# michael-fonder/M4Depth

Hardware: AMD Instinct MI355X
Metric: frames/s (higher is better)
Workload: dtype f32

## Files before the change

### m4depth_amd/csrc/m4d_reduce.hip

```cpp
#include <cstdlib>
#include "m4d_common.h"
#include "../../include/m4depth_hip.h"

namespace {

constexpr int kDinlMaxBlocks = 512;
__host__ __device__ constexpr long long dinl_partial_floats(int b, int C) { return 2LL * b * kDinlMaxBlocks * C; }

__global__ void __launch_bounds__(256)
dinl_partial_kernel(const float* __restrict__ x, const float* __restrict__ mean, int hw, int C, int pass,
                    double* __restrict__ partial) {
  __shared__ double sh[4][256];
  const int bi = blockIdx.y;
  const int c4n = C >> 2;
  const int ppi = 256 / c4n;
  const int c4 = threadIdx.x % c4n, po = threadIdx.x / c4n;
  const float* xb = x + (long long)bi * hw * C;
  float4 m = make_float4(0.f, 0.f, 0.f, 0.f);
  if (pass == 1) m = *reinterpret_cast<const float4*>(mean + bi * C + c4 * 4);
  double acc[4] = {0.0, 0.0, 0.0, 0.0};
  for (int p = blockIdx.x * ppi + po; p < hw; p += gridDim.x * ppi) {
    float4 v = *reinterpret_cast<const float4*>(xb + (long long)p * C + c4 * 4);
    if (pass == 1) {
      v.x = v.x - m.x; v.y = v.y - m.y; v.z = v.z - m.z; v.w = v.w - m.w;
      v.x = v.x * v.x; v.y = v.y * v.y; v.z = v.z * v.z; v.w = v.w * v.w;
    }
    acc[0] += (double)v.x; acc[1] += (double)v.y; acc[2] += (double)v.z; acc[3] += (double)v.w;
  }
#pragma unroll
  for (int e = 0; e < 4; ++e) sh[e][threadIdx.x] = acc[e];
  __syncthreads();
  if (po == 0) {
    double* pp = partial + ((long long)bi * gridDim.x + blockIdx.x) * C + c4 * 4;
#pragma unroll
    for (int e = 0; e < 4; ++e) {
      double s = sh[e][c4];
      for (int r = 1; r < ppi; ++r) s += sh[e][r * c4n + c4];
      pp[e] = s;
    }
  }
}

__global__ void __launch_bounds__(256)
dinl_finalize_kernel(const double* __restrict__ partial, int nblk, int C, int hw, float* __restrict__ out) {
  __shared__ double sh[256];
  const int bi = blockIdx.x;
  const int c = threadIdx.x % C, j = threadIdx.x / C, nj = 256 / C;
  double s = 0.0;
  for (int k = j; k < nblk; k += nj) s += partial[((long long)bi * nblk + k) * C + c];
  sh[threadIdx.x] = s;
  __syncthreads();
  if (j == 0) {
    for (int r = 1; r < nj; ++r) s += sh[r * C + c];
    out[bi * C + c] = (float)(s / (double)hw);
  }
}

template <int C>
__global__ void __launch_bounds__(256)
dinl_apply_kernel(const float* __restrict__ x, const float* __restrict__ mean, const float* __restrict__ var,
                  const float* __restrict__ scale, const float* __restrict__ bias, int hw, int w, float slope,
                  float* __restrict__ out, int out_h, int out_w, int off_y, int off_x) {
  const int bi = blockIdx.y;
  float mu[C], dv[C], sc[C], bs[C];
#pragma unroll
  for (int c = 0; c < C; ++c) {
    mu[c] = mean[bi * C + c];
    dv[c] = var[bi * C + c] + 1e-12f;
    sc[c] = scale[c];
    bs[c] = bias[c];
  }
  for (int p = blockIdx.x * blockDim.x + threadIdx.x; p < hw; p += gridDim.x * blockDim.x) {
    const float* px = x + ((long long)bi * hw + p) * C;
    float n[C];
    float ss = 0.f;
#pragma unroll
    for (int c = 0; c < C; c += 4) {
      const float4 v = *reinterpret_cast<const float4*>(px + c);
      n[c] = (v.x - mu[c]) / dv[c]; n[c + 1] = (v.y - mu[c + 1]) / dv[c + 1];
      n[c + 2] = (v.z - mu[c + 2]) / dv[c + 2]; n[c + 3] = (v.w - mu[c + 3]) / dv[c + 3];
    }
#pragma unroll
    for (int c = 0; c < C; ++c) ss = ss + n[c] * n[c];
    const float inv = 1.0f / sqrtf(fmaxf(ss, 1e-12f));
    float* po = out + (((long long)bi * out_h + (p / w + off_y)) * out_w + (p % w + off_x)) * C;
#pragma unroll
    for (int c = 0; c < C; c += 4) {
      float4 o;
      o.x = sc[c] * (n[c] * inv) + bs[c]; o.y = sc[c + 1] * (n[c + 1] * inv) + bs[c + 1];
      o.z = sc[c + 2] * (n[c + 2] * inv) + bs[c + 2]; o.w = sc[c + 3] * (n[c + 3] * inv) + bs[c + 3];
      o.x = o.x > 0.f ? o.x : o.x * slope; o.y = o.y > 0.f ? o.y : o.y * slope;
      o.z = o.z > 0.f ? o.z : o.z * slope; o.w = o.w > 0.f ? o.w : o.w * slope;
      *reinterpret_cast<float4*>(po + c) = o;
    }
  }
}

template <int C>
__global__ void __launch_bounds__(256)
enc_head_conv_kernel(const float* __restrict__ img, const float* __restrict__ w27, const float* __restrict__ bias,
                     int h, int w, int bsz, long long stride_b, long long stride_t,
                     float* __restrict__ out, double* __restrict__ partial) {
  __shared__ double sh[4][C];
  const int bi = blockIdx.y;
  const int hw = h * w;
  const float* ib = img + (long long)(bi % bsz) * stride_b + (long long)(bi / bsz) * stride_t;
  float* ob = out + (long long)bi * hw * C;
  double csum[C];
#pragma unroll
  for (int c = 0; c < C; ++c) csum[c] = 0.0;
  for (int p = blockIdx.x * 256 + threadIdx.x; p < hw; p += gridDim.x * 256) {
    const int y = p / w, x = p - y * w;
    typedef float f2 __attribute__((ext_vector_type(2)));
    f2 acc2[C / 2];
#pragma unroll
    for (int c = 0; c < C / 2; ++c) acc2[c] = (f2){0.f, 0.f};
#pragma unroll
    for (int ky = 0; ky < 3; ++ky) {
      const int yy = y + ky - 1;
#pragma unroll
      for (int kx = 0; kx < 3; ++kx) {
        const int xx = x + kx - 1;
        const bool in = yy >= 0 && yy < h && xx >= 0 && xx < w;
        const float* px = ib + ((long long)(in ? yy : y) * w + (in ? xx : x)) * 3;
        const float v0 = in ? px[0] : 0.f, v1 = in ? px[1] : 0.f, v2 = in ? px[2] : 0.f;
        const f2* wt = reinterpret_cast<const f2*>(w27 + (ky * 3 + kx) * 3 * C);
#pragma unroll
        for (int c = 0; c < C / 2; ++c)
          acc2[c] = ((acc2[c] + (f2){v0, v0} * wt[c]) + (f2){v1, v1} * wt[C / 2 + c]) + (f2){v2, v2} * wt[C + c];
      }
    }
    float acc[C];
#pragma unroll
    for (int c = 0; c < C / 2; ++c) { acc[2 * c] = acc2[c].x; acc[2 * c + 1] = acc2[c].y; }
#pragma unroll
    for (int c = 0; c < C; c += 4) {
      float4 o = make_float4(acc[c] + bias[c], acc[c + 1] + bias[c + 1], acc[c + 2] + bias[c + 2], acc[c + 3] + bias[c + 3]);
      *reinterpret_cast<float4*>(ob + (long long)p * C + c) = o;
      csum[c] += (double)o.x; csum[c + 1] += (double)o.y; csum[c + 2] += (double)o.z; csum[c + 3] += (double)o.w;
    }
  }
#pragma unroll
  for (int c = 0; c < C; ++c) {
    double v = csum[c];
#pragma unroll
    for (int o = 32; o > 0; o >>= 1) v += __shfl_xor(v, o);
    if ((threadIdx.x & 63) == 0) sh[threadIdx.x >> 6][c] = v;
  }
  __syncthreads();
  if (threadIdx.x < C)
    partial[((long long)bi * gridDim.x + blockIdx.x) * C + threadIdx.x] =
        ((sh[0][threadIdx.x] + sh[1][threadIdx.x]) + sh[2][threadIdx.x]) + sh[3][threadIdx.x];
}

constexpr int kMetricSums = 9;
constexpr int kMetricBlocks = 512;

__global__ void __launch_bounds__(256)
metrics_partial_kernel(const float* __restrict__ gt_raw, const float* __restrict__ est_raw, long long n, float max_d,
                       double* __restrict__ partial, long long per_image, long long gt_image_stride) {
  float s[kMetricSums];
#pragma unroll
  for (int k = 0; k < kMetricSums; ++k) s[k] = 0.f;
  const long long step = (long long)gridDim.x * blockDim.x;
  long long i = (long long)blockIdx.x * blockDim.x + threadIdx.x;
  long long img = i / per_image, off = i - img * per_image;
  for (; i < n; i += step) {
    const float gt = fminf(fmaxf(gt_raw[img * gt_image_stride + off], 0.0f), max_d);
    off += step;
    while (off >= per_image) { off -= per_image; ++img; }
    const float est = fminf(fmaxf(est_raw[i], 0.001f), max_d);
    const bool m = gt > 1e-6f;
    const float diff = gt - est;
    const float lg = logf(gt + 1e-6f), le = logf(est + 1e-6f);
    const bool m2 = lg > 1e-6f;
    const float th = fmaxf(gt / est, est / gt);
    if (m) {
      s[0] += 1.0f;
      s[1] += fabsf(diff) / (gt + 1e-6f);
      s[2] += diff * diff / (gt + 1e-6f);
      s[3] += diff * diff;
      s[6] += th < 1.25f ? 1.0f : 0.0f;
      s[7] += th < 1.5625f ? 1.0f : 0.0f;
      s[8] += th < 1.953125f ? 1.0f : 0.0f;
    }
    if (m2) { s[4] += 1.0f; s[5] += (lg - le) * (lg - le); }
  }
  __shared__ double sh[4][kMetricSums];
#pragma unroll
  for (int k = 0; k < kMetricSums; ++k) {
    double v = (double)s[k];
#pragma unroll
    for (int o = 32; o > 0; o >>= 1) v += __shfl_down(v, o);
    if ((threadIdx.x & 63) == 0) sh[threadIdx.x >> 6][k] = v;
  }
  __syncthreads();
  if (threadIdx.x < kMetricSums)
    partial[(long long)blockIdx.x * kMetricSums + threadIdx.x] =
        ((sh[0][threadIdx.x] + sh[1][threadIdx.x]) + sh[2][threadIdx.x]) + sh[3][threadIdx.x];
}

__global__ void __launch_bounds__(kMetricSums * 32)
metrics_finalize_kernel(const double* __restrict__ partial, int nblk, float* __restrict__ out7,
                        float* __restrict__ total7, float count, float* __restrict__ mean7) {
  __shared__ double sub[kMetricSums * 32];
  __shared__ double tot[kMetricSums];
  const int q = threadIdx.x % kMetricSums, j = threadIdx.x / kMetricSums;
  double s = 0.0;
  for (int k = j; k < nblk; k += 32) s += partial[(long long)k * kMetricSums + q];
  sub[threadIdx.x] = s;
  __syncthreads();
  if (j == 0) {
    for (int r = 1; r < 32; ++r) s += sub[r * kMetricSums + q];
    tot[q] = s;
  }
  __syncthreads();
  if (threadIdx.x == 0) {
    const double cnt = tot[0] > 1.0 ? tot[0] : 1.0, cnt2 = tot[4] > 1.0 ? tot[4] : 1.0;
    out7[0] = (float)(tot[1] / cnt);
    out7[1] = (float)(tot[2] / cnt);
    out7[2] = sqrtf((float)(tot[3] / cnt));
    out7[3] = sqrtf((float)(tot[5] / cnt2));
    out7[4] = (float)(tot[6] / cnt);
    out7[5] = (float)(tot[7] / cnt);
    out7[6] = (float)(tot[8] / cnt);
    if (total7) {
#pragma unroll
      for (int i = 0; i < 7; ++i) {
        const float t = total7[i] + out7[i];
        total7[i] = t;
        if (mean7) mean7[i] = t / count;
      }
    }
  }
}

__global__ void __launch_bounds__(256)
metrics_partial_ps_kernel(const float* __restrict__ gt_raw, long long gt_stride, const float* __restrict__ est_raw,
                          long long est_stride, long long n, float max_d, double* __restrict__ partial) {
  const float* gt_img = gt_raw + (long long)blockIdx.y * gt_stride;
  const float* est_img = est_raw + (long long)blockIdx.y * est_stride;
  float s[kMetricSums];
#pragma unroll
  for (int k = 0; k < kMetricSums; ++k) s[k] = 0.f;
  const long long step = (long long)gridDim.x * blockDim.x;
  for (long long i = (long long)blockIdx.x * blockDim.x + threadIdx.x; i < n; i += step) {
    const float gt = fminf(fmaxf(gt_img[i], 0.0f), max_d);
    const float est = fminf(fmaxf(est_img[i], 0.001f), max_d);
    const bool m = gt > 1e-6f;
    const float diff = gt - est;
    const float lg = logf(gt + 1e-6f), le = logf(est + 1e-6f);
    const bool m2 = lg > 1e-6f;
    const float th = fmaxf(gt / est, est / gt);
    if (m) {
      s[0] += 1.0f;
      s[1] += fabsf(diff) / (gt + 1e-6f);
      s[2] += diff * diff / (gt + 1e-6f);
      s[3] += diff * diff;
      s[6] += th < 1.25f ? 1.0f : 0.0f;
      s[7] += th < 1.5625f ? 1.0f : 0.0f;
      s[8] += th < 1.953125f ? 1.0f : 0.0f;
    }
    if (m2) { s[4] += 1.0f; s[5] += (lg - le) * (lg - le); }
  }
  __shared__ double sh[4][kMetricSums];
#pragma unroll
  for (int k = 0; k < kMetricSums; ++k) {
    double v = (double)s[k];
#pragma unroll
    for (int o = 32; o > 0; o >>= 1) v += __shfl_down(v, o);
    if ((threadIdx.x & 63) == 0) sh[threadIdx.x >> 6][k] = v;
  }
  __syncthreads();
  if (threadIdx.x < kMetricSums)
    partial[((long long)blockIdx.y * gridDim.x + blockIdx.x) * kMetricSums + threadIdx.x] =
        ((sh[0][threadIdx.x] + sh[1][threadIdx.x]) + sh[2][threadIdx.x]) + sh[3][threadIdx.x];
}

__global__ void __launch_bounds__(kMetricSums * 32)
metrics_finalize_ps_kernel(const double* __restrict__ partial, int nblk, const unsigned char* __restrict__ new_traj,
                           const unsigned char* __restrict__ active, float* __restrict__ rows, unsigned char* __restrict__ counted) {
  __shared__ double sub[kMetricSums * 32];
  __shared__ double tot[kMetricSums];
  const int smp = blockIdx.x;
  const double* pp = partial + (long long)smp * nblk * kMetricSums;
  const int q = threadIdx.x % kMetricSums, j = threadIdx.x / kMetricSums;
  double s = 0.0;
  for (int k = j; k < nblk; k += 32) s += pp[(long long)k * kMetricSums + q];
  sub[threadIdx.x] = s;
  __syncthreads();
  if (j == 0) {
    for (int r = 1; r < 32; ++r) s += sub[r * kMetricSums + q];
    tot[q] = s;
  }
  __syncthreads();
  if (threadIdx.x == 0) {
    const double cnt = tot[0] > 1.0 ? tot[0] : 1.0, cnt2 = tot[4] > 1.0 ? tot[4] : 1.0;
    float* out7 = rows + (long long)smp * 7;
    out7[0] = (float)(tot[1] / cnt);
    out7[1] = (float)(tot[2] / cnt);
    out7[2] = sqrtf((float)(tot[3] / cnt));
    out7[3] = sqrtf((float)(tot[5] / cnt2));
    out7[4] = (float)(tot[6] / cnt);
    out7[5] = (float)(tot[7] / cnt);
    out7[6] = (float)(tot[8] / cnt);
    counted[smp] = (active[smp] != 0 && new_traj[smp] == 0) ? 1 : 0;
  }
}


typedef float f32x4 __attribute__((ext_vector_type(4)));

__device__ __forceinline__ void enc0_lane_setup(const float* __restrict__ w27, int lane, int row_stride, int (&koff)[7], float (&wb)[7]) {
  const int j = lane & 15, g = lane >> 4;
#pragma unroll
  for (int s = 0; s < 7; ++s) {
    const int k = 4 * s + g;
    const bool valid = k < 27;
    const int kk = valid ? k : 0;
    koff[s] = (kk / 9) * row_stride + kk % 9;
    wb[s] = valid ? w27[k * 16 + j] : 0.f;
  }
}
__device__ __forceinline__ f32x4 enc0_conv1(const float* window_base, const int (&koff)[7], const float (&wb)[7]) {
  f32x4 acc = {0.f, 0.f, 0.f, 0.f};
#pragma unroll
  for (int s = 0; s < 7; ++s) acc = __builtin_amdgcn_mfma_f32_16x16x4f32(window_base[koff[s]], wb[s], acc, 0, 0, 0);
  return acc;
}

constexpr int kE0TW = 128, kE0TH = 8;
constexpr int kE0RS = (kE0TW + 2) * 3;

__device__ __forceinline__ float enc0_shift(const float* __restrict__ ib, const float* __restrict__ w27, const float* __restrict__ bias,
                                            int h, int w, int j) {
  const int cy = h / 2, cx = w / 2;
  float y = bias[j];
  for (int ky = 0; ky < 3; ++ky)
    for (int kx = 0; kx < 3; ++kx) {
      const int gy = cy + ky - 1, gx = cx + kx - 1;
      if (gy < 0 || gy >= h || gx < 0 || gx >= w) continue;
      for (int ch = 0; ch < 3; ++ch) y = y + w27[((ky * 3 + kx) * 3 + ch) * 16 + j] * ib[((long long)gy * w + gx) * 3 + ch];
    }
  return y;
}

template <int PASS>
__global__ void __launch_bounds__(256)
enc0_stats_kernel(const float* __restrict__ img, const float* __restrict__ w27, const float* __restrict__ bias,
                  const float* __restrict__ mean, int h, int w, int bsz, long long stride_b, long long stride_t,
                  int tiles_x, int n_tiles, double* __restrict__ partial) {
  __shared__ float tile[(kE0TH + 2) * kE0RS];
  __shared__ double sh[2][4][16];
  const int t = threadIdx.x, lane = t & 63, wv = t >> 6;
  const int j = lane & 15, g = lane >> 4;
  const int bi = blockIdx.y;
  const float* ib = img + (long long)(bi % bsz) * stride_b + (long long)(bi / bsz) * stride_t;
  int koff[7]; float wb[7];
  enc0_lane_setup(w27, lane, kE0RS, koff, wb);
  const float bias_j = bias[j];
  const float mean_j = PASS == 1 ? mean[bi * 16 + j] : (PASS == 2 ? enc0_shift(ib, w27, bias, h, w, j) : 0.f);
  const double shift_j = (double)mean_j;
  double csum = 0.0, csum2 = 0.0;
  for (int ti = blockIdx.x; ti < n_tiles; ti += gridDim.x) {
    const int y0 = (ti / tiles_x) * kE0TH, x0 = (ti % tiles_x) * kE0TW;
    __syncthreads();
    for (int idx = t; idx < (kE0TH + 2) * kE0RS; idx += 256) {
      const int r = idx / kE0RS, cc = idx - r * kE0RS;
      const int gy = y0 - 1 + r, gxc = (x0 - 1) * 3 + cc;
      const bool in = gy >= 0 && gy < h && gxc >= 0 && gxc < w * 3;
      tile[idx] = in ? ib[(long long)gy * w * 3 + gxc] : 0.f;
    }
    __syncthreads();
#pragma unroll
    for (int rr = 0; rr < 2; ++rr) {
      const int yl = 2 * wv + rr;
#pragma unroll
      for (int ct = 0; ct < kE0TW / 16; ++ct) {
        const f32x4 acc = enc0_conv1(tile + yl * kE0RS + 3 * (16 * ct + j), koff, wb);
#pragma unroll
        for (int r = 0; r < 4; ++r) {
          const bool valid = y0 + yl < h && x0 + 16 * ct + 4 * g + r < w;
          float v = acc[r] + bias_j;
          if (PASS == 1) { v = v - mean_j; v = v * v; }
          if (PASS == 2) {
            const double d = valid ? (double)v - shift_j : 0.0;
            csum += d;
            csum2 = fma(d, d, csum2);
          } else {
            csum += valid ? (double)v : 0.0;
          }
        }
      }
    }
  }
  csum += __shfl_xor(csum, 16);
  csum += __shfl_xor(csum, 32);
  if (PASS == 2) {
    csum2 += __shfl_xor(csum2, 16);
    csum2 += __shfl_xor(csum2, 32);
  }
  if (lane < 16) { sh[0][wv][lane] = csum; sh[1][wv][lane] = csum2; }
  __syncthreads();
  constexpr int NQ = PASS == 2 ? 32 : 16;
  if (t < NQ) {
    const int q = t >> 4, c = t & 15;
    partial[((long long)bi * gridDim.x + blockIdx.x) * NQ + t] = ((sh[q][0][c] + sh[q][1][c]) + sh[q][2][c]) + sh[q][3][c];
  }
}

__global__ void __launch_bounds__(256)
enc0_moments_finalize_kernel(const float* __restrict__ img, const double* __restrict__ partial, int nblk, const float* __restrict__ w27,
                             const float* __restrict__ bias, int h, int w, int bsz, long long stride_b, long long stride_t,
                             float* __restrict__ mean, float* __restrict__ var) {
  __shared__ double sh[256];
  const int bi = blockIdx.x, t = threadIdx.x;
  const int c = t & 31, j = t >> 5;
  double pv[32];
  const int cnt = (nblk - j + 7) / 8;
#pragma unroll
  for (int i = 0; i < 32; ++i) pv[i] = i < cnt ? partial[((long long)bi * nblk + j + 8 * i) * 32 + c] : 0.0;
  __shared__ float s_shift[16];
  if (t >= 240) {
    const float* ib0 = img + (long long)(bi % bsz) * stride_b + (long long)(bi / bsz) * stride_t;
    s_shift[t - 240] = enc0_shift(ib0, w27, bias, h, w, t - 240);
  }
  double s = 0.0;
#pragma unroll
  for (int i = 0; i < 32; ++i) s += pv[i];
  sh[t] = s;
  __syncthreads();
  if (t < 32) {
    for (int r = 1; r < 8; ++r) s += sh[r * 32 + t];
    sh[t] = s;
  }
  __syncthreads();
  if (t < 16) {
    const double n = (double)h * (double)w;
    const double m1 = sh[t] / n, m2 = sh[16 + t] / n;
    mean[bi * 16 + t] = (float)((double)s_shift[t] + m1);
    const double v = m2 - m1 * m1;
    var[bi * 16 + t] = (float)(v > 0.0 ? v : 0.0);
  }
}

__global__ void __launch_bounds__(256)
enc0_rgb_total_kernel(const float* __restrict__ img, int hw, int bsz, long long stride_b, long long stride_t, float* __restrict__ partial) {
  __shared__ float sh[4][3];
  const int t = threadIdx.x, bi = blockIdx.y;
  const float* ib = img + (long long)(bi % bsz) * stride_b + (long long)(bi / bsz) * stride_t;
  float s0 = 0.f, s1 = 0.f, s2 = 0.f;
  for (int p = blockIdx.x * 256 + t; p < hw; p += gridDim.x * 256) {
    s0 += ib[(long long)p * 3]; s1 += ib[(long long)p * 3 + 1]; s2 += ib[(long long)p * 3 + 2];
  }
#pragma unroll
  for (int o = 32; o > 0; o >>= 1) { s0 += __shfl_xor(s0, o); s1 += __shfl_xor(s1, o); s2 += __shfl_xor(s2, o); }
  if ((t & 63) == 0) { sh[t >> 6][0] = s0; sh[t >> 6][1] = s1; sh[t >> 6][2] = s2; }
  __syncthreads();
  if (t < 3) partial[((long long)bi * gridDim.x + blockIdx.x) * 3 + t] = ((sh[0][t] + sh[1][t]) + sh[2][t]) + sh[3][t];
}

__global__ void __launch_bounds__(256)
enc0_mean_kernel(const float* __restrict__ img, const float* __restrict__ partial, int nblk, const float* __restrict__ w27,
                 const float* __restrict__ bias, int h, int w, int bsz, long long stride_b, long long stride_t, float* __restrict__ mean) {
  __shared__ double red[15][256];
  __shared__ double sums[3][5];
  const int t = threadIdx.x, bi = blockIdx.x;
  const float* ib = img + (long long)(bi % bsz) * stride_b + (long long)(bi / bsz) * stride_t;
  double acc[15];
#pragma unroll
  for (int q = 0; q < 15; ++q) acc[q] = 0.0;
  for (int k = t; k < nblk; k += 256)
#pragma unroll
    for (int ch = 0; ch < 3; ++ch) acc[ch * 5] += (double)partial[((long long)bi * nblk + k) * 3 + ch];
  for (int x = t; x < w; x += 256)
#pragma unroll
    for (int ch = 0; ch < 3; ++ch) {
      acc[ch * 5 + 1] += (double)ib[(long long)x * 3 + ch];
      acc[ch * 5 + 2] += (double)ib[((long long)(h - 1) * w + x) * 3 + ch];
    }
  for (int y = t; y < h; y += 256)
#pragma unroll
    for (int ch = 0; ch < 3; ++ch) {
      acc[ch * 5 + 3] += (double)ib[((long long)y * w) * 3 + ch];
      acc[ch * 5 + 4] += (double)ib[((long long)y * w + (w - 1)) * 3 + ch];
    }
#pragma unroll
  for (int q = 0; q < 15; ++q) red[q][t] = acc[q];
  __syncthreads();
  for (int o = 128; o > 0; o >>= 1) {
    if (t < o)
#pragma unroll
      for (int q = 0; q < 15; ++q) red[q][t] += red[q][t + o];
    __syncthreads();
  }
  if (t < 15) sums[t / 5][t % 5] = red[t][0];
  __syncthreads();
  if (t < 16) {
    double m = 0.0;
    for (int ky = 0; ky < 3; ++ky)
      for (int kx = 0; kx < 3; ++kx)
        for (int ch = 0; ch < 3; ++ch) {
          const int ry = ky == 0 ? h - 1 : (ky == 2 ? 0 : -1), cx = kx == 0 ? w - 1 : (kx == 2 ? 0 : -1);
          double sv = sums[ch][0];
          if (ry >= 0) sv -= sums[ch][ry == 0 ? 1 : 2];
          if (cx >= 0) sv -= sums[ch][cx == 0 ? 3 : 4];
          if (ry >= 0 && cx >= 0) sv += (double)ib[((long long)ry * w + cx) * 3 + ch];
          m += (double)w27[((ky * 3 + kx) * 3 + ch) * 16 + t] * sv;
        }
    mean[bi * 16 + t] = (float)((double)bias[t] + m / ((double)h * (double)w));
  }
}

#ifndef M4D_E0_ABL
#define M4D_E0_ABL 0
#endif
constexpr int kF0OW = 16, kF0OH = 8;
constexpr int kF0CW = 2 * kF0OW + 1, kF0CH = 2 * kF0OH + 1;
constexpr int kF0RW = kF0CW + 2, kF0RH = kF0CH + 2;
constexpr int kF0RS = kF0RW * 3;
constexpr int kF0NS = 17;
constexpr int kF0NP = kF0CW * kF0CH;

__device__ __forceinline__ bool v_dummy(float x) { return x != 1.2345e-30f; }
__global__ void __launch_bounds__(256)
enc0_fused_kernel(const float* __restrict__ img, const float* __restrict__ w27, const float* __restrict__ bias1,
                  const float* __restrict__ mean, const float* __restrict__ var, const float* __restrict__ dn_scale,
                  const float* __restrict__ dn_bias, float dn_slope, const float* __restrict__ w2, const float* __restrict__ bias2,
                  float slope, int h, int w, int oh, int ow, int pad_y, int pad_x, int bsz, long long stride_b, long long stride_t,
                  int tiles_x, float* __restrict__ out) {
  __shared__ float rgb[kF0RH * kF0RS];
  __shared__ float nrm[kF0NP * kF0NS];
  const int t = threadIdx.x, lane = t & 63, wv = t >> 6;
  const int j = lane & 15, g = lane >> 4;
  const int bi = blockIdx.y;
  const float* ib = img + (long long)(bi % bsz) * stride_b + (long long)(bi / bsz) * stride_t;
  const int oy0 = (blockIdx.x / tiles_x) * kF0OH, ox0 = (blockIdx.x % tiles_x) * kF0OW;
  const int cy0 = 2 * oy0 - pad_y, cx0 = 2 * ox0 - pad_x;
  for (int idx = t; idx < kF0RH * kF0RS; idx += 256) {
    const int r = idx / kF0RS, cc = idx - r * kF0RS;
    const int gy = cy0 - 1 + r, gxc = (cx0 - 1) * 3 + cc;
    const bool in = gy >= 0 && gy < h && gxc >= 0 && gxc < w * 3;
    rgb[idx] = (in && !(M4D_E0_ABL & 1)) ? ib[(long long)gy * w * 3 + gxc] : 0.f;
  }
  int koff[7]; float wb[7];
  enc0_lane_setup(w27, lane, kF0RS, koff, wb);
  const float bias_j = bias1[j];
  __shared__ float s_mu[16], s_dv[16], s_sc[16], s_bs[16];
  if (t < 16) {
    s_mu[t] = mean[bi * 16 + t];
    s_dv[t] = 1.0f / (var[bi * 16 + t] + 1e-12f);
    s_sc[t] = dn_scale[t]; s_bs[t] = dn_bias[t];
  }
  float wb2[36];
#pragma unroll
  for (int s = 0; s < 36; ++s) wb2[s] = w2[(4 * s + g) * 16 + j];
  const float bias2_j = bias2[j];
  __syncthreads();
  static_assert((kF0NP + 15) / 16 == 36, "nine 16-pixel tiles per wave");
#pragma unroll 3
  for (int it = 0; it < 9; ++it) {
    const int tl = wv + 4 * it;
    const int pa = min(16 * tl + j, kF0NP - 1);
    const int ay = pa / kF0CW, ax = pa - ay * kF0CW;
    const f32x4 acc = (M4D_E0_ABL & 2) ? f32x4{wb[0], wb[1], wb[2], wb[3]} : enc0_conv1(rgb + ay * kF0RS + 3 * ax, koff, wb);
#pragma unroll
    for (int r = 0; r < 4; ++r) {
      const int p = 16 * tl + 4 * g + r;
      if (p < kF0NP) nrm[p * kF0NS + j] = acc[r] + bias_j;
    }
  }
  __syncthreads();
  for (int p = t; p < ((M4D_E0_ABL & 4) ? 0 : kF0NP); p += 256) {
    const int py = p / kF0CW, px = p - py * kF0CW;
    const bool inside = cy0 + py >= 0 && cy0 + py < h && cx0 + px >= 0 && cx0 + px < w;
    float* q = nrm + p * kF0NS;
    float n[16];
    float ss = 0.f;
#pragma unroll
    for (int c = 0; c < 16; ++c) { n[c] = (q[c] - s_mu[c]) * s_dv[c]; ss = ss + n[c] * n[c]; }
    const float inv = 1.0f / sqrtf(fmaxf(ss, 1e-12f));
#pragma unroll
    for (int c = 0; c < 16; ++c) {
      float o = s_sc[c] * (n[c] * inv) + s_bs[c];
      o = o > 0.f ? o : o * dn_slope;
      q[c] = inside ? o : 0.f;
    }
  }
  __syncthreads();
#pragma unroll
  for (int rr = 0; rr < 2; ++rr) {
    const int oyl = 2 * wv + rr;
    const float* base = nrm + ((2 * oyl) * kF0CW + 2 * j) * kF0NS + g;
    f32x4 acc = {0.f, 0.f, 0.f, 0.f};
#pragma unroll
    for (int s = 0; s < ((M4D_E0_ABL & 8) ? 1 : 36); ++s) {
      const int tap = s >> 2, ky = tap / 3, kx = tap - 3 * ky;
      acc = __builtin_amdgcn_mfma_f32_16x16x4f32(base[(ky * kF0CW + kx) * kF0NS + 4 * (s & 3)], wb2[s], acc, 0, 0, 0);
    }
    const int oy = oy0 + oyl;
#pragma unroll
    for (int r = 0; r < 4; ++r) {
      const int ox = ox0 + 4 * g + r;
      if (oy < oh && ox < ow && !((M4D_E0_ABL & 16) && v_dummy(acc[r]))) {
        float v = acc[r] + bias2_j;
        v = v > 0.f ? v : v * slope;
        out[(((long long)bi * oh + oy) * ow + ox) * 16 + j] = v;
      }
    }
  }
}

}

extern "C" long long m4d_dinl_workspace_floats(int b, int C) {
  return dinl_partial_floats(b, C) + 2LL * b * C;
}

extern "C" int m4d_dinl_fwd(const float* x, const float* scale, const float* bias, int b, int h, int w, int C,
                            float slope, float* workspace, float* out, void* stream) {
  return m4d_dinl_fwd_padded(x, scale, bias, b, h, w, C, slope, workspace, out, h, w, 0, 0, stream);
}

extern "C" int m4d_dinl_fwd_padded(const float* x, const float* scale, const float* bias, int b, int h, int w, int C,
                                   float slope, float* workspace, float* out, int out_h, int out_w, int off_y,
                                   int off_x, void* stream) {
  M4D_CHECK_ARG(x && scale && bias && workspace && out && b > 0 && h > 0 && w > 0);
  M4D_CHECK_ARG(off_y >= 0 && off_x >= 0 && off_y + h <= out_h && off_x + w <= out_w);
  M4D_CHECK_ARG(C == 16 || C == 32);
  M4D_CHECK_ARG(((((uintptr_t)x | (uintptr_t)out | (uintptr_t)workspace)) & 15u) == 0);
  hipStream_t s = (hipStream_t)stream;
  const int hw = h * w;
  const int ppi = 256 / (C / 4);
  int nblk = (hw + ppi * 8 - 1) / (ppi * 8);
  if (nblk > kDinlMaxBlocks) nblk = kDinlMaxBlocks;
  double* partial = reinterpret_cast<double*>(workspace);
  float* mean = workspace + dinl_partial_floats(b, C);
  float* var = mean + (long long)b * C;
  m4d_launch(dinl_partial_kernel, dim3(nblk, b), dim3(256), 0, s, x, (const float*)nullptr, hw, C, 0, partial);
  m4d_launch(dinl_finalize_kernel, dim3(b), dim3(256), 0, s, (const double*)partial, nblk, C, hw, mean);
  m4d_launch(dinl_partial_kernel, dim3(nblk, b), dim3(256), 0, s, x, (const float*)mean, hw, C, 1, partial);
  m4d_launch(dinl_finalize_kernel, dim3(b), dim3(256), 0, s, (const double*)partial, nblk, C, hw, var);
  int gx = m4d_blocks(hw, 256);
  if (gx > 2048) gx = 2048;
  if (C == 16) m4d_launch(dinl_apply_kernel<16>, dim3(gx, b), dim3(256), 0, s, x, mean, var, scale, bias, hw, w, slope, out, out_h, out_w, off_y, off_x);
  else m4d_launch(dinl_apply_kernel<32>, dim3(gx, b), dim3(256), 0, s, x, mean, var, scale, bias, hw, w, slope, out, out_h, out_w, off_y, off_x);
  return M4D_LAUNCH_RESULT();
}

extern "C" int m4d_enc_head_fwd(const float* images, int bsz, long long stride_b, long long stride_t,
                                const float* w_hwio, const float* bias, int b, int h, int w, int C,
                                float* workspace, float* raw_out, void* stream) {
  M4D_CHECK_ARG(images && w_hwio && bias && workspace && raw_out && b > 0 && h > 0 && w > 0);
  M4D_CHECK_ARG(C == 16);
  M4D_CHECK_ARG(bsz > 0 && b % bsz == 0 && stride_b >= 0 && stride_t >= 0);
  M4D_CHECK_ARG(((((uintptr_t)raw_out | (uintptr_t)workspace)) & 15u) == 0);
  hipStream_t s = (hipStream_t)stream;
  const int hw = h * w;
  int nblk = (hw + 256 * 8 - 1) / (256 * 8);
  if (nblk > kDinlMaxBlocks) nblk = kDinlMaxBlocks;
  if (nblk < 1) nblk = 1;
  double* partial = reinterpret_cast<double*>(workspace);
  float* mean = workspace + dinl_partial_floats(b, C);
  float* var = mean + (long long)b * C;
  m4d_launch(enc_head_conv_kernel<16>, dim3(nblk, b), dim3(256), 0, s, images, w_hwio, bias, h, w, bsz, stride_b, stride_t,
                     raw_out, partial);
  m4d_launch(dinl_finalize_kernel, dim3(b), dim3(256), 0, s, (const double*)partial, nblk, C, hw, mean);
  const int ppi = 256 / (C / 4);
  int nblk2 = (hw + ppi * 8 - 1) / (ppi * 8);
  if (nblk2 > kDinlMaxBlocks) nblk2 = kDinlMaxBlocks;
  m4d_launch(dinl_partial_kernel, dim3(nblk2, b), dim3(256), 0, s, (const float*)raw_out, (const float*)mean, hw, C, 1, partial);
  m4d_launch(dinl_finalize_kernel, dim3(b), dim3(256), 0, s, (const double*)partial, nblk2, C, hw, var);
  return M4D_LAUNCH_RESULT();
}

extern "C" int m4d_enc_level0_stats(const float* images, int bsz, long long stride_b, long long stride_t,
                                    const float* w1_hwio, const float* bias1, int b, int h, int w, float* workspace,
                                    float* mean, float* var, void* stream) {
  M4D_CHECK_ARG(images && w1_hwio && bias1 && workspace && mean && var);
  M4D_CHECK_ARG(b > 0 && h > 0 && w > 0 && bsz > 0 && b % bsz == 0 && stride_b >= 0 && stride_t >= 0);
  M4D_CHECK_ARG((((uintptr_t)workspace) & 7u) == 0);
  hipStream_t s = (hipStream_t)stream;
  const int C = 16, hw = h * w;
  const int tiles_x = (w + kE0TW - 1) / kE0TW, n_tiles = tiles_x * ((h + kE0TH - 1) / kE0TH);
  const int nblk = n_tiles < kDinlMaxBlocks ? n_tiles : kDinlMaxBlocks;
  double* partial = reinterpret_cast<double*>(workspace);
  static const int single_pass = [] { const char* e = getenv("M4D_ENC0_SINGLE_PASS"); return e ? atoi(e) : 1; }();
  static const int analytic_mean_env = [] { const char* e = getenv("M4D_ENC0_ANALYTIC_MEAN"); return e ? atoi(e) : 1; }();
  if (single_pass) {
    const int cap = kDinlMaxBlocks / 2, per = (n_tiles + cap - 1) / cap;
    const int nb2 = (n_tiles + per - 1) / per;
    m4d_launch(enc0_stats_kernel<2>, dim3(nb2, b), dim3(256), 0, s, images, w1_hwio, bias1, (const float*)nullptr, h, w, bsz,
               stride_b, stride_t, tiles_x, n_tiles, partial);
    m4d_launch(enc0_moments_finalize_kernel, dim3(b), dim3(256), 0, s, images, (const double*)partial, nb2, w1_hwio, bias1, h, w, bsz,
               stride_b, stride_t, mean, var);
    return M4D_LAUNCH_RESULT();
  }
  const bool analytic_mean = analytic_mean_env && h > 1 && w > 1;
  if (analytic_mean) {
    int nb3 = (hw + 256 * 16 - 1) / (256 * 16);
    if (nb3 > kDinlMaxBlocks) nb3 = kDinlMaxBlocks;
    m4d_launch(enc0_rgb_total_kernel, dim3(nb3, b), dim3(256), 0, s, images, hw, bsz, stride_b, stride_t, workspace);
    m4d_launch(enc0_mean_kernel, dim3(b), dim3(256), 0, s, images, (const float*)workspace, nb3, w1_hwio, bias1, h, w, bsz,
                       stride_b, stride_t, mean);
  } else {
    m4d_launch(enc0_stats_kernel<0>, dim3(nblk, b), dim3(256), 0, s, images, w1_hwio, bias1, (const float*)nullptr, h, w, bsz,
                       stride_b, stride_t, tiles_x, n_tiles, partial);
    m4d_launch(dinl_finalize_kernel, dim3(b), dim3(256), 0, s, (const double*)partial, nblk, C, hw, mean);
  }
  m4d_launch(enc0_stats_kernel<1>, dim3(nblk, b), dim3(256), 0, s, images, w1_hwio, bias1, (const float*)mean, h, w, bsz,
                     stride_b, stride_t, tiles_x, n_tiles, partial);
  m4d_launch(dinl_finalize_kernel, dim3(b), dim3(256), 0, s, (const double*)partial, nblk, C, hw, var);
  return M4D_LAUNCH_RESULT();
}

extern "C" int m4d_enc_level0_apply(const float* images, int bsz, long long stride_b, long long stride_t,
                                    const float* w1_hwio, const float* bias1, const float* mean, const float* var,
                                    const float* dn_scale, const float* dn_bias, float dn_slope, const float* w2_hwio,
                                    const float* bias2, float slope, int b, int h, int w, float* out, void* stream) {
  M4D_CHECK_ARG(images && w1_hwio && bias1 && mean && var && dn_scale && dn_bias && w2_hwio && bias2 && out);
  M4D_CHECK_ARG(b > 0 && h > 0 && w > 0 && bsz > 0 && b % bsz == 0 && stride_b >= 0 && stride_t >= 0);
  const int oh = (h + 1) / 2, ow = (w + 1) / 2;
  const int ftx = (ow + kF0OW - 1) / kF0OW, fty = (oh + kF0OH - 1) / kF0OH;
  const int tot_y = (oh - 1) * 2 + 3 - h, tot_x = (ow - 1) * 2 + 3 - w;
  const int pad_y = (tot_y > 0 ? tot_y : 0) / 2, pad_x = (tot_x > 0 ? tot_x : 0) / 2;
  m4d_launch(enc0_fused_kernel, dim3(ftx * fty, b), dim3(256), 0, (hipStream_t)stream, images, w1_hwio, bias1, mean,
                     var, dn_scale, dn_bias, dn_slope, w2_hwio, bias2, slope, h, w, oh, ow, pad_y, pad_x, bsz, stride_b,
                     stride_t, ftx, out);
  return M4D_LAUNCH_RESULT();
}

extern "C" int m4d_enc_level0_fwd(const float* images, int bsz, long long stride_b, long long stride_t,
                                   const float* w1_hwio, const float* bias1, const float* dn_scale, const float* dn_bias,
                                   float dn_slope, const float* w2_hwio, const float* bias2, float slope,
                                   int b, int h, int w, float* workspace, float* out, void* stream) {
  M4D_CHECK_ARG(workspace && b > 0);
  float* mean = workspace + dinl_partial_floats(b, 16);
  float* var = mean + (long long)b * 16;
  const int rc = m4d_enc_level0_stats(images, bsz, stride_b, stride_t, w1_hwio, bias1, b, h, w, workspace, mean, var, stream);
  if (rc != 0) return rc;
  return m4d_enc_level0_apply(images, bsz, stride_b, stride_t, w1_hwio, bias1, mean, var, dn_scale, dn_bias, dn_slope, w2_hwio,
                              bias2, slope, b, h, w, out, stream);
}

extern "C" long long m4d_metrics_workspace_bytes(void) { return (long long)kMetricBlocks * kMetricSums * sizeof(double); }

extern "C" int m4d_depth_metrics_strided(const float* gt, long long per_image, long long gt_image_stride, const float* est,
                                         long long n, float max_d, void* workspace, float* out7, float* total7, float count,
                                         float* mean7, void* stream) {
  M4D_CHECK_ARG(gt && est && workspace && out7 && n > 0 && per_image > 0 && gt_image_stride >= per_image && n % per_image == 0);
  M4D_CHECK_ARG(!mean7 || (total7 && count > 0.f));
  hipStream_t s = (hipStream_t)stream;
  long long g = (n + 255) / 256;
  const int nblk = (int)(g < kMetricBlocks ? g : kMetricBlocks);
  m4d_launch(metrics_partial_kernel, dim3(nblk), dim3(256), 0, s, gt, est, n, max_d, (double*)workspace, per_image, gt_image_stride);
  m4d_launch(metrics_finalize_kernel, dim3(1), dim3(kMetricSums * 32), 0, s, (const double*)workspace, nblk, out7, total7, count, mean7);
  return M4D_LAUNCH_RESULT();
}

extern "C" int m4d_depth_metrics(const float* gt, const float* est, long long n, float max_d, void* workspace,
                                 float* out7, float* total7, float count, float* mean7, void* stream) {
  return m4d_depth_metrics_strided(gt, n, n, est, n, max_d, workspace, out7, total7, count, mean7, stream);
}

extern "C" long long m4d_metrics_per_sample_workspace_bytes(int b) {
  return b > 0 ? (long long)b * kMetricBlocks * kMetricSums * sizeof(double) : 0;
}

extern "C" int m4d_depth_metrics_per_sample(const float* gt, long long gt_stride, const float* est, long long est_stride,
                                            int b, long long per_image, float max_d, const unsigned char* new_traj,
                                            const unsigned char* active, void* workspace, float* rows, unsigned char* counted,
                                            void* stream) {
  M4D_CHECK_ARG(gt && est && new_traj && active && workspace && rows && counted);
  M4D_CHECK_ARG(b > 0 && b <= 65535 && per_image > 0 && gt_stride >= per_image && est_stride >= per_image);
  hipStream_t s = (hipStream_t)stream;
  long long g = (per_image + 255) / 256;
  const int nblk = (int)(g < kMetricBlocks ? g : kMetricBlocks);
  m4d_launch(metrics_partial_ps_kernel, dim3(nblk, b), dim3(256), 0, s, gt, gt_stride, est, est_stride, per_image, max_d,
             (double*)workspace);
  m4d_launch(metrics_finalize_ps_kernel, dim3(b), dim3(kMetricSums * 32), 0, s, (const double*)workspace, nblk, new_traj, active,
             rows, counted);
  return M4D_LAUNCH_RESULT();
}
```

Before: 1791.

## Double-buffer enc0 stats tiles and interleave MFMA chains in fused first layer

The stats kernel now double-buffers its shared-memory input tile. Each thread prefetches the next tile's pixels into registers while the current tile's MFMA convolution runs, which removes one barrier per iteration, and a compile-time fast path skips the bounds checks for interior tiles. The shift computation is split into a load phase and a sum phase so its global loads are issued early, and the finalize kernel computes the shift in every thread instead of a separate branch. In the fused encoder kernel, global loads go into registers before the stores to LDS, three independent MFMA chains are interleaved in the first conv, and the second conv's two rows are computed together with software-prefetched LDS operands and scheduling barriers. The cost is higher register pressure, which could reduce occupancy.

Result: faster. 1814 (median of 6 runs) (+1.3%).

```diff
diff --git a/m4depth_amd/csrc/m4d_reduce.hip b/m4depth_amd/csrc/m4d_reduce.hip
--- a/m4depth_amd/csrc/m4d_reduce.hip
+++ b/m4depth_amd/csrc/m4d_reduce.hip
@@ -1,3 +1,4 @@
+#include <type_traits>
 #include <cstdlib>
 #include "m4d_common.h"
 #include "../../include/m4depth_hip.h"
@@ -329,20 +330,66 @@
   return acc;
 }
 
+#ifndef M4D_E0S_ABL
+#define M4D_E0S_ABL 0
+#endif
 constexpr int kE0TW = 128, kE0TH = 8;
 constexpr int kE0RS = (kE0TW + 2) * 3;
 
-__device__ __forceinline__ float enc0_shift(const float* __restrict__ ib, const float* __restrict__ w27, const float* __restrict__ bias,
-                                            int h, int w, int j) {
+__device__ __forceinline__ void enc0_shift_load(const float* __restrict__ ib, const float* __restrict__ w27, int h, int w, int j,
+                                                float (&sw)[27], float (&sp)[27]) {
   const int cy = h / 2, cx = w / 2;
-  float y = bias[j];
+#pragma unroll
   for (int ky = 0; ky < 3; ++ky)
+#pragma unroll
     for (int kx = 0; kx < 3; ++kx) {
       const int gy = cy + ky - 1, gx = cx + kx - 1;
-      if (gy < 0 || gy >= h || gx < 0 || gx >= w) continue;
-      for (int ch = 0; ch < 3; ++ch) y = y + w27[((ky * 3 + kx) * 3 + ch) * 16 + j] * ib[((long long)gy * w + gx) * 3 + ch];
+      const bool ok = !(gy < 0 || gy >= h || gx < 0 || gx >= w);
+      const long long base = ok ? ((long long)gy * w + gx) * 3 : 0LL;
+#pragma unroll
+      for (int ch = 0; ch < 3; ++ch) {
+        sw[(ky * 3 + kx) * 3 + ch] = w27[((ky * 3 + kx) * 3 + ch) * 16 + j];
+        sp[(ky * 3 + kx) * 3 + ch] = ib[base + ch];
+      }
+    }
+}
+__device__ __forceinline__ float enc0_shift_sum(float bias_j, const float (&sw)[27], const float (&sp)[27], int h, int w) {
+  const int cy = h / 2, cx = w / 2;
+  float y = bias_j;
+#pragma unroll
+  for (int ky = 0; ky < 3; ++ky)
+#pragma unroll
+    for (int kx = 0; kx < 3; ++kx) {
+      const int gy = cy + ky - 1, gx = cx + kx - 1;
+      const bool ok = !(gy < 0 || gy >= h || gx < 0 || gx >= w);
+#pragma unroll
+      for (int ch = 0; ch < 3; ++ch) y = ok ? y + sw[(ky * 3 + kx) * 3 + ch] * sp[(ky * 3 + kx) * 3 + ch] : y;
     }
   return y;
+}
+
+constexpr int kE0TE = (kE0TH + 2) * kE0RS;
+constexpr int kE0NL = (kE0TE + 255) / 256;
+static_assert(kE0RS > 256 && kE0RS < 512, "enc0_tile_load: thread t starts in row 0 and crosses at most one row end per step of 256");
+__device__ __forceinline__ unsigned enc0_tile_load(const float* __restrict__ ib, int h, int w, int y0, int x0, int t, float (&v)[kE0NL]) {
+  const int row3 = w * 3, gy0 = y0 - 1, gc0 = (x0 - 1) * 3;
+  int r = 0, cc = t;
+  unsigned mask = 0u;
+#pragma unroll
+  for (int i = 0; i < kE0NL; ++i) {
+    const int gy = gy0 + r, gxc = gc0 + cc;
+    const bool in = r < kE0TH + 2 && gy >= 0 && gy < h && gxc >= 0 && gxc < row3;
+    v[i] = ib[(long long)min(max(gy, 0), h - 1) * row3 + min(max(gxc, 0), row3 - 1)];
+    mask |= in ? 1u << i : 0u;
+    cc += 256;
+    if (cc >= kE0RS) { cc -= kE0RS; ++r; }
+  }
+  return mask;
+}
+__device__ __forceinline__ void enc0_tile_store(float* __restrict__ tile, int t, const float (&v)[kE0NL], unsigned mask) {
+#pragma unroll
+  for (int i = 0; i < kE0NL; ++i)
+    if (t + 256 * i < kE0TE) tile[t + 256 * i] = (mask >> i & 1u) ? v[i] : 0.f;
 }
 
 template <int PASS>
@@ -350,49 +397,65 @@
 enc0_stats_kernel(const float* __restrict__ img, const float* __restrict__ w27, const float* __restrict__ bias,
                   const float* __restrict__ mean, int h, int w, int bsz, long long stride_b, long long stride_t,
                   int tiles_x, int n_tiles, double* __restrict__ partial) {
-  __shared__ float tile[(kE0TH + 2) * kE0RS];
+  __shared__ float tile[2][kE0TE];
   __shared__ double sh[2][4][16];
   const int t = threadIdx.x, lane = t & 63, wv = t >> 6;
   const int j = lane & 15, g = lane >> 4;
   const int bi = blockIdx.y;
   const float* ib = img + (long long)(bi % bsz) * stride_b + (long long)(bi / bsz) * stride_t;
+  float v[kE0NL];
+  int ti = blockIdx.x;
+  unsigned vmask = 0u;
+  if (ti < n_tiles) vmask = enc0_tile_load(ib, h, w, (ti / tiles_x) * kE0TH, (ti % tiles_x) * kE0TW, t, v);
+  float sw[27], sp[27];
+  if (PASS == 2) enc0_shift_load(ib, w27, h, w, j, sw, sp);
   int koff[7]; float wb[7];
   enc0_lane_setup(w27, lane, kE0RS, koff, wb);
   const float bias_j = bias[j];
-  const float mean_j = PASS == 1 ? mean[bi * 16 + j] : (PASS == 2 ? enc0_shift(ib, w27, bias, h, w, j) : 0.f);
+  const float mean_j = PASS == 1 ? mean[bi * 16 + j] : (PASS == 2 ? enc0_shift_sum(bias_j, sw, sp, h, w) : 0.f);
   const double shift_j = (double)mean_j;
   double csum = 0.0, csum2 = 0.0;
-  for (int ti = blockIdx.x; ti < n_tiles; ti += gridDim.x) {
+  if (ti < n_tiles) enc0_tile_store(tile[0], t, v, vmask);
+  __syncthreads();
+  int cur = 0;
+  for (; ti < n_tiles; ti += gridDim.x) {
     const int y0 = (ti / tiles_x) * kE0TH, x0 = (ti % tiles_x) * kE0TW;
-    __syncthreads();
-    for (int idx = t; idx < (kE0TH + 2) * kE0RS; idx += 256) {
-      const int r = idx / kE0RS, cc = idx - r * kE0RS;
-      const int gy = y0 - 1 + r, gxc = (x0 - 1) * 3 + cc;
-      const bool in = gy >= 0 && gy < h && gxc >= 0 && gxc < w * 3;
-      tile[idx] = in ? ib[(long long)gy * w * 3 + gxc] : 0.f;
-    }
-    __syncthreads();
-#pragma unroll
-    for (int rr = 0; rr < 2; ++rr) {
-      const int yl = 2 * wv + rr;
-#pragma unroll
-      for (int ct = 0; ct < kE0TW / 16; ++ct) {
-        const f32x4 acc = enc0_conv1(tile + yl * kE0RS + 3 * (16 * ct + j), koff, wb);
-#pragma unroll
-        for (int r = 0; r < 4; ++r) {
-          const bool valid = y0 + yl < h && x0 + 16 * ct + 4 * g + r < w;
-          float v = acc[r] + bias_j;
-          if (PASS == 1) { v = v - mean_j; v = v * v; }
-          if (PASS == 2) {
-            const double d = valid ? (double)v - shift_j : 0.0;
-            csum += d;
-            csum2 = fma(d, d, csum2);
-          } else {
-            csum += valid ? (double)v : 0.0;
+    const int tn = ti + gridDim.x;
+    const bool more = tn < n_tiles;
+    if (more) vmask = enc0_tile_load(ib, h, w, (tn / tiles_x) * kE0TH, (tn % tiles_x) * kE0TW, t, v);
+    const float* tb = tile[cur];
+    auto tile_sums = [&](auto whole) {
+      constexpr bool kWhole = decltype(whole)::value;
+#pragma unroll 1
+      for (int rr = 0; rr < 2; ++rr) {
+        const int yl = 2 * wv + rr;
+#pragma unroll 4
+        for (int ct = 0; ct < kE0TW / 16; ++ct) {
+          const float* wnd = tb + yl * kE0RS + 3 * (16 * ct + j);
+          const f32x4 acc = (M4D_E0S_ABL & 2) ? f32x4{wnd[koff[0]], wnd[koff[1]], wnd[koff[2]], wnd[koff[3]]} : enc0_conv1(wnd, koff, wb);
+#pragma unroll
+          for (int r = 0; r < 4; ++r) {
+            const bool valid = kWhole || (y0 + yl < h && x0 + 16 * ct + 4 * g + r < w);
+            float v1 = acc[r] + bias_j;
+            if (M4D_E0S_ABL & 4) { csum += r == 0 ? (double)v1 : 0.0; continue; }
+            if (PASS == 1) { v1 = v1 - mean_j; v1 = v1 * v1; }
+            if (PASS == 2) {
+              const double d = valid ? (double)v1 - shift_j : 0.0;
+              csum += d;
+              csum2 = fma(d, d, csum2);
+            } else {
+              csum += valid ? (double)v1 : 0.0;
+            }
           }
         }
       }
-    }
+    };
+    if (y0 + kE0TH <= h && x0 + kE0TW <= w) tile_sums(std::true_type{}); else tile_sums(std::false_type{});
+    if (more) {
+      enc0_tile_store(tile[cur ^ 1], t, v, vmask);
+      __syncthreads();
+    }
+    cur ^= 1;
   }
   csum += __shfl_xor(csum, 16);
   csum += __shfl_xor(csum, 32);
@@ -416,15 +479,18 @@
   __shared__ double sh[256];
   const int bi = blockIdx.x, t = threadIdx.x;
   const int c = t & 31, j = t >> 5;
+  const float* ib0 = img + (long long)(bi % bsz) * stride_b + (long long)(bi / bsz) * stride_t;
+  float sw[27], sp[27];
+  enc0_shift_load(ib0, w27, h, w, t & 15, sw, sp);
+  const float sbias = bias[t & 15];
   double pv[32];
   const int cnt = (nblk - j + 7) / 8;
 #pragma unroll
-  for (int i = 0; i < 32; ++i) pv[i] = i < cnt ? partial[((long long)bi * nblk + j + 8 * i) * 32 + c] : 0.0;
-  __shared__ float s_shift[16];
-  if (t >= 240) {
-    const float* ib0 = img + (long long)(bi % bsz) * stride_b + (long long)(bi / bsz) * stride_t;
-    s_shift[t - 240] = enc0_shift(ib0, w27, bias, h, w, t - 240);
-  }
+  for (int i = 0; i < 32; ++i) {
+    const double x = partial[i < cnt ? ((long long)bi * nblk + j + 8 * i) * 32 + c : 0LL];
+    pv[i] = i < cnt ? x : 0.0;
+  }
+  const float shift = enc0_shift_sum(sbias, sw, sp, h, w);
   double s = 0.0;
 #pragma unroll
   for (int i = 0; i < 32; ++i) s += pv[i];
@@ -438,7 +504,7 @@
   if (t < 16) {
     const double n = (double)h * (double)w;
     const double m1 = sh[t] / n, m2 = sh[16 + t] / n;
-    mean[bi * 16 + t] = (float)((double)s_shift[t] + m1);
+    mean[bi * 16 + t] = (float)((double)shift + m1);
     const double v = m2 - m1 * m1;
     var[bi * 16 + t] = (float)(v > 0.0 ? v : 0.0);
   }
@@ -537,37 +603,74 @@
   const float* ib = img + (long long)(bi % bsz) * stride_b + (long long)(bi / bsz) * stride_t;
   const int oy0 = (blockIdx.x / tiles_x) * kF0OH, ox0 = (blockIdx.x % tiles_x) * kF0OW;
   const int cy0 = 2 * oy0 - pad_y, cx0 = 2 * ox0 - pad_x;
-  for (int idx = t; idx < kF0RH * kF0RS; idx += 256) {
-    const int r = idx / kF0RS, cc = idx - r * kF0RS;
-    const int gy = cy0 - 1 + r, gxc = (cx0 - 1) * 3 + cc;
-    const bool in = gy >= 0 && gy < h && gxc >= 0 && gxc < w * 3;
-    rgb[idx] = (in && !(M4D_E0_ABL & 1)) ? ib[(long long)gy * w * 3 + gxc] : 0.f;
+  constexpr int kNL = (kF0RH * kF0RS + 255) / 256, kStep = 256 - 2 * kF0RS;
+  static_assert(kStep >= 0 && kStep < kF0RS && 3 * kF0RS > 256, "the row / column walk below");
+  float sv[kNL];
+  {
+    const int row3 = w * 3, gy0 = cy0 - 1, gc0 = (cx0 - 1) * 3;
+    int r = (t >= kF0RS) + (t >= 2 * kF0RS), cc = t - r * kF0RS;
+#pragma unroll
+    for (int i = 0; i < kNL; ++i) {
+      const int gy = gy0 + r, gxc = gc0 + cc;
+      const bool in = r < kF0RH && gy >= 0 && gy < h && gxc >= 0 && gxc < row3 && !(M4D_E0_ABL & 1);
+      const float x = ib[in ? (long long)gy * row3 + gxc : 0LL];
+      sv[i] = in ? x : 0.f;
+      r += 2; cc += kStep;
+      if (cc >= kF0RS) { cc -= kF0RS; ++r; }
+    }
   }
   int koff[7]; float wb[7];
   enc0_lane_setup(w27, lane, kF0RS, koff, wb);
   const float bias_j = bias1[j];
   __shared__ float s_mu[16], s_dv[16], s_sc[16], s_bs[16];
-  if (t < 16) {
-    s_mu[t] = mean[bi * 16 + t];
-    s_dv[t] = 1.0f / (var[bi * 16 + t] + 1e-12f);
-    s_sc[t] = dn_scale[t]; s_bs[t] = dn_bias[t];
-  }
+  const float st_mu = mean[bi * 16 + (t & 15)], st_var = var[bi * 16 + (t & 15)], st_sc = dn_scale[t & 15], st_bs = dn_bias[t & 15];
   float wb2[36];
 #pragma unroll
   for (int s = 0; s < 36; ++s) wb2[s] = w2[(4 * s + g) * 16 + j];
   const float bias2_j = bias2[j];
-  __syncthreads();
-  static_assert((kF0NP + 15) / 16 == 36, "nine 16-pixel tiles per wave");
-#pragma unroll 3
-  for (int it = 0; it < 9; ++it) {
-    const int tl = wv + 4 * it;
-    const int pa = min(16 * tl + j, kF0NP - 1);
-    const int ay = pa / kF0CW, ax = pa - ay * kF0CW;
-    const f32x4 acc = (M4D_E0_ABL & 2) ? f32x4{wb[0], wb[1], wb[2], wb[3]} : enc0_conv1(rgb + ay * kF0RS + 3 * ax, koff, wb);
+#pragma unroll
+  for (int i = 0; i < kNL; ++i)
+    if (t + 256 * i < kF0RH * kF0RS) rgb[t + 256 * i] = sv[i];
+  if (t < 16) {
+    s_mu[t] = st_mu;
+    s_dv[t] = 1.0f / (st_var + 1e-12f);
+    s_sc[t] = st_sc; s_bs[t] = st_bs;
+  }
+  __syncthreads();
+  static_assert((kF0NP + 15) / 16 == 36 && kF0NP > 16 * 35, "nine 16-pixel tiles per wave, the last one of wave 3 ragged");
+#pragma unroll 1
+  for (int it = 0; it < 9; it += 3) {
+    const float* wa[3];
+#pragma unroll
+    for (int u = 0; u < 3; ++u) {
+      const int pa = min(16 * (wv + 4 * (it + u)) + j, kF0NP - 1);
+      const int ay = pa / kF0CW, ax = pa - ay * kF0CW;
+      wa[u] = rgb + ay * kF0RS + 3 * ax;
+    }
+    f32x4 c0 = {0.f, 0.f, 0.f, 0.f}, c1 = c0, c2 = c0;
+    if (M4D_E0_ABL & 2) {
+      c0 = c1 = c2 = f32x4{wb[0], wb[1], wb[2], wb[3]};
+    } else {
+#pragma unroll
+      for (int s = 0; s < 7; ++s) {
+        c0 = __builtin_amdgcn_mfma_f32_16x16x4f32(wa[0][koff[s]], wb[s], c0, 0, 0, 0);
+        c1 = __builtin_amdgcn_mfma_f32_16x16x4f32(wa[1][koff[s]], wb[s], c1, 0, 0, 0);
+        c2 = __builtin_amdgcn_mfma_f32_16x16x4f32(wa[2][koff[s]], wb[s], c2, 0, 0, 0);
+      }
+    }
+    float* n0 = nrm + (16 * (wv + 4 * it) + 4 * g) * kF0NS + j;
 #pragma unroll
     for (int r = 0; r < 4; ++r) {
-      const int p = 16 * tl + 4 * g + r;
-      if (p < kF0NP) nrm[p * kF0NS + j] = acc[r] + bias_j;
+      n0[r * kF0NS] = c0[r] + bias_j;
+      n0[(64 + r) * kF0NS] = c1[r] + bias_j;
+    }
+    if (it < 6 || wv < 3) {
+#pragma unroll
+      for (int r = 0; r < 4; ++r) n0[(128 + r) * kF0NS] = c2[r] + bias_j;
+    } else {
+#pragma unroll
+      for (int r = 0; r < 4; ++r)
+        if (16 * 35 + 4 * g + r < kF0NP) n0[(128 + r) * kF0NS] = c2[r] + bias_j;
     }
   }
   __syncthreads();
@@ -588,16 +691,27 @@
     }
   }
   __syncthreads();
+  constexpr int kS2 = (M4D_E0_ABL & 8) ? 1 : 36;
+  const float* base2 = nrm + ((4 * wv) * kF0CW + 2 * j) * kF0NS + g;
+  auto a2 = [&](int rr, int s) {
+    const int tap = s >> 2, ky = tap / 3, kx = tap - 3 * ky;
+    return base2[((2 * rr + ky) * kF0CW + kx) * kF0NS + 4 * (s & 3)];
+  };
+  f32x4 acc2[2] = {{0.f, 0.f, 0.f, 0.f}, {0.f, 0.f, 0.f, 0.f}};
+  float xa[2][2] = {{a2(0, 0), a2(1, 0)}, {a2(0, kS2 > 1 ? 1 : 0), a2(1, kS2 > 1 ? 1 : 0)}};
+#pragma unroll
+  for (int s = 0; s < kS2; ++s) {
+    const float x0 = xa[s & 1][0], x1 = xa[s & 1][1];
+    if (s + 2 < kS2) { xa[s & 1][0] = a2(0, s + 2); xa[s & 1][1] = a2(1, s + 2); }
+    acc2[0] = __builtin_amdgcn_mfma_f32_16x16x4f32(x0, wb2[s], acc2[0], 0, 0, 0);
+    acc2[1] = __builtin_amdgcn_mfma_f32_16x16x4f32(x1, wb2[s], acc2[1], 0, 0, 0);
+    __builtin_amdgcn_sched_group_barrier(0x100, 2, 0);
+    __builtin_amdgcn_sched_group_barrier(0x008, 2, 0);
+  }
 #pragma unroll
   for (int rr = 0; rr < 2; ++rr) {
     const int oyl = 2 * wv + rr;
-    const float* base = nrm + ((2 * oyl) * kF0CW + 2 * j) * kF0NS + g;
-    f32x4 acc = {0.f, 0.f, 0.f, 0.f};
-#pragma unroll
-    for (int s = 0; s < ((M4D_E0_ABL & 8) ? 1 : 36); ++s) {
-      const int tap = s >> 2, ky = tap / 3, kx = tap - 3 * ky;
-      acc = __builtin_amdgcn_mfma_f32_16x16x4f32(base[(ky * kF0CW + kx) * kF0NS + 4 * (s & 3)], wb2[s], acc, 0, 0, 0);
-    }
+    const f32x4 acc = acc2[rr];
     const int oy = oy0 + oyl;
 #pragma unroll
     for (int r = 0; r < 4; ++r) {
```
